# jnhansen/nd

Measured on AMD Instinct MI355X. Metric: Mpixels/s OmnibusTest dual-pol 24t x 4096 x 4096, higher is better.
Workload: dtype f32; 1 GPU; OmnibusTest C2 24t x 4096 x 4096 f32 per GPU (BASELINE configs[1]), resident in HBM; looks=9, rows_per_rank=4096

## Files before the change

nd_amd/build.py:

```python
import os
import subprocess
import sys

HERE = os.path.dirname(os.path.abspath(__file__))
CSRC = os.path.join(HERE, 'csrc')
OBJ = os.path.join(CSRC, '_build')
LIB = os.path.join(HERE, 'libnd_amd.so')
HIPCC = os.environ.get('HIPCC', '/opt/rocm/bin/hipcc')
ARCH = 'gfx950'

FLAGS = ['--offload-arch=' + ARCH, '-O3', '-std=c++17', '-fPIC', '-ffp-contract=off',
         '-fno-fast-math', '-Wall', '-Wno-unused-function']


PER_FILE = {'nlmeans.hip': ['-fno-slp-vectorize'],
            'omnibus.hip': ['-fno-slp-vectorize'],
            'omnibus_c3.hip': ['-fno-slp-vectorize'],
            'omnibus_ml.hip': ['-fno-slp-vectorize'],
            'omnibus_diag.hip': ['-fno-slp-vectorize']}


NO_SCRATCH = {'omnibus_ml.hip': 'omnibus_c2_ml_kernel', 'rgb.hip': 'rgb_', 'classify.hip': 'class',
              'kmeans_fit.hip': '_kernel', 'omnibus_diag.hip': 'omnibus_diag_',
              'change_segments.hip': 'change_segments_kernel', 'rasterize.hip': 'rasterize_', 'resample.hip': 'resample_',
              'speckle.hip': 'speckle_'}
SCRATCH_BUDGET = {(False, False): 0, (False, True): 96, (True, False): 256, (True, True): 384}


def _template_bools(mangled, symbol):
    import re
    m = re.search(re.escape(symbol) + r'I((?:L[ib]\d+E)+)E', mangled)
    if not m:
        return None
    flags = re.findall(r'Lb(\d)E', m.group(1))
    return (flags[0] == '1', flags[1] == '1') if len(flags) == 2 else None


def check_no_scratch(remarks_path, symbol, obj_path=None):
    import re
    if not os.path.exists(remarks_path) or (obj_path and os.path.exists(obj_path)
                                            and os.path.getmtime(remarks_path) + 1.0 < os.path.getmtime(obj_path)):
        return []
    found, cur = [], None
    for ln in open(remarks_path, errors='replace'):
        m = re.search(r'Function Name: (\S+)', ln)
        if m:
            cur = m.group(1)
            continue
        m = re.search(r'ScratchSize \[bytes/lane\]: (\d+)', ln)
        if m and cur is not None and symbol in cur:
            found.append((cur, int(m.group(1))))
    strict = os.environ.get('ND_AMD_STRICT_SCRATCH', '') == '1'
    if not found:
        msg = ('%s: no resource report for %s (is -Rpass-analysis=kernel-resource-usage on?)'
               % (remarks_path, symbol))
        if strict:
            raise RuntimeError(msg)
        sys.stderr.write('nd_amd.build: warning: ' + msg + '\n')
        return found
    bad = []
    for f, n in found:
        key = _template_bools(f, symbol)
        budget = SCRATCH_BUDGET.get(key, 0) if key is not None else 0
        if n > budget:
            bad.append((f, n, budget))
    if bad:
        msg = 'scratch use (bytes per lane) over budget: %s' % bad
        if strict:
            raise RuntimeError(msg)
        sys.stderr.write('nd_amd.build: warning: ' + msg + ' (speed only; ND_AMD_STRICT_SCRATCH=1 makes this an error)\n')
    return found


def sources():
    return sorted(os.path.join(CSRC, f) for f in os.listdir(CSRC) if f.endswith('.hip'))
# ... 71 lines not shown
```

nd_amd/csrc/omnibus.hip:

```cpp
#include <type_traits>

#include "dispatch.hpp"
#include "omnibus_c2_device.hpp"

namespace nd_amd {

template <typename T, int PPT, bool STATS>
__global__ void __launch_bounds__(kGlobalThreads)
omnibus_c2_global_kernel(const OmniGlobalArgs<T> g, const OmniTab tab)
{
    const int tid = threadIdx.x;
    const int lane = tid & 63;
    const int64_t b = blockIdx.x;
    const int64_t row = b / g.blocks_per_row;
    const int64_t bx = b - row * g.blocks_per_row;
    const int64_t bpx0 = bx * (int64_t)(kGlobalThreads * PPT);
    const int64_t x0 = bpx0 + (int64_t)tid * PPT;
    const int k = g.k;

    if (g.write_tab && b == 0) {
        for (int j = tid; j <= k; j += kGlobalThreads) g.tab_dev[j] = tab.e[j];
    }

    {
// ... 129 lines not shown
    const int64_t bpx0 = bx * (int64_t)kRetainThreads;
    const int64_t x0 = bpx0 + tid;
    const int k = g.k;
    const bool in = x0 < g.nx;

    T v[KMAX][4];
    retain_load_series<T, KMAX, EXACT>(g, row, bpx0, tid, in, k, v);

    if (g.write_tab && b == 0) {
        for (int j = tid; j <= k; j += kRetainThreads) g.tab_dev[j] = tab.e[j];
    }

    Accum<T> A;
    A.reset();
#pragma unroll
    for (int t = 0; t < KMAX; ++t)
        if (EXACT || t < k) A.step(v[t][0], v[t][1], v[t][2], v[t][3]);

    bool flag;
    if (STATS) {
        flag = global_flag_stats<T>(z_stat<T>(A, k, g.nlooks, g.e), 4 * (k - 1), g.e, g.alpha, in, g.z_out, g.p_out,
                                    row * g.nx + x0);
    } else {
        flag = in && (z_approx<T>(A, k, g.nlooks, g.e) >= g.e.zlo_a);
    }

    const unsigned long long m = __ballot(flag);
    const bool dense_wave = __popcll(m) >= g.dense_min;
    if (m != 0ull) {
        const unsigned shard = (unsigned)(b % kShards);
        if (dense_wave) {
            if (lane == 0) {
                const unsigned slot = atomicAdd(g.flag_count + shard * kCounterStride + 1, 1u);
                g.dense_idx[(size_t)shard * g.segd + slot] = (uint32_t)(row * g.nx + bpx0 + (tid & ~63));
            }
        } else {
            const unsigned slot = wave_claim(flag, g.flag_count + shard * kCounterStride, lane);
            if (flag) {
                g.flag_idx[(size_t)shard * g.seg + slot] = (uint32_t)(row * g.nx + x0);
                if (slot < g.dump_cap)
                    dump_series<T, KMAX, EXACT>(g.dump + ((int64_t)shard * g.dump_cap + slot) * (int64_t)(4 * k), v, k);
            }
        }
    }

    {
        const int64_t left = g.nx - bpx0;
        const int npx = left > kRetainThreads ? kRetainThreads : (int)left;
        zero_fill_span<kRetainThreads>(g.change + (row * g.nx + bpx0) * (int64_t)k, npx * k, tid);
    }
}

template <typename T, int KMAX, bool EXACT>
__global__ void __launch_bounds__(kRetainThreads, 4)
omnibus_c2_retain_wsearch_kernel(const OmniGlobalArgs<T> g, const OmniTab tab, const DenseScreen fscr)
{
    static_assert(KMAX % 4 == 0 && KMAX <= 24, "rows of whole words; 4 KMAX series registers within four waves per SIMD");
    constexpr int kWaves = kRetainThreads / 64;
    __shared__ __align__(16) T series_img[kWaves][kWaveSearchMax * KMAX * 4];
    __shared__ __align__(4) uint8_t rows_img[kWaves][kWaveSearchMax * KMAX];
    static_assert(sizeof(series_img[0]) >= 16 * KMAX * sizeof(uint32_t), "store_change_rows_wave's image");
    const int tid = threadIdx.x;
    const int lane = tid & 63;
    const int64_t b = blockIdx.x;
    const int64_t row = b / g.blocks_per_row;
    const int64_t bx = b - row * g.blocks_per_row;
    const int64_t bpx0 = bx * (int64_t)kRetainThreads;
    const int64_t x0 = bpx0 + tid;
    const int k = EXACT ? KMAX : g.k;
    const bool in = x0 < g.nx;

    T v[KMAX][4];
    retain_load_series<T, KMAX, EXACT>(g, row, bpx0, tid, in, k, v);

    if (g.write_tab && b == 0) {
        for (int j = tid; j <= k; j += kRetainThreads) g.tab_dev[j] = tab.e[j];
    }

    Accum<T> A;
    A.reset();
#pragma unroll
    for (int t = 0; t < KMAX; ++t)
        if (EXACT || t < k) A.step(v[t][0], v[t][1], v[t][2], v[t][3]);
    const bool flag = in && (z_approx<T>(A, k, g.nlooks, g.e) >= g.e.zlo_a);

    const unsigned long long m = __ballot(flag);
    const int nc = __popcll(m);
    const int64_t wpx0 = bpx0 + (tid & ~63);
    const int64_t wleft = g.nx - wpx0;
    const int wnp = wleft > 64 ? 64 : (wleft > 0 ? (int)wleft : 0);
    uint8_t *wob = g.change + (row * g.nx + wpx0) * (int64_t)k;

    if (nc == 0 || nc > kWaveSearchMax) {
        if (nc != 0 && lane == 0) {
            const unsigned shard = (unsigned)(b % kShards);
            const unsigned slot = atomicAdd(g.flag_count + shard * kCounterStride + 1, 1u);
            g.dense_idx[(size_t)shard * g.segd + slot] = (uint32_t)(row * g.nx + wpx0);
        }
        if (wnp > 0) zero_fill_span(wob, wnp * k, lane);
        return;
    }

    T *img = series_img[tid >> 6];
    uint8_t *rows = rows_img[tid >> 6];
    uint32_t *rows_w = reinterpret_cast<uint32_t *>(rows);
    const int rank = __popcll(m & ((1ull << lane) - 1ull));
    if (flag) dump_series<T, KMAX, EXACT>(img + rank * (KMAX * 4), v, k);
    for (int w = lane; w < kWaveSearchMax * KMAX / 4; w += 64) rows_w[w] = 0u;
    asm volatile("s_waitcnt lgkmcnt(0)" ::: "memory");
    wave_search_starts<T, KMAX>(img, rows, nc, k, g.nlooks, g.alpha, fscr.e, tab.e, lane);
    asm volatile("s_waitcnt lgkmcnt(0)" ::: "memory");
    unsigned mask = 0u;
    if (flag) {
#pragma unroll
        for (int q = 0; q < KMAX / 4; ++q)
            mask |= (((rows_w[rank * (KMAX / 4) + q] * 0x01020408u) >> 24) & 0xFu) << (4 * q);
    }
    if (change_rows_wave_ok(wob, k, wnp)) {
        store_change_rows_wave(wob, reinterpret_cast<uint32_t *>(img), k, mask, lane);
    } else if (in) {
        store_change_row_lane<KMAX>(wob + (int64_t)lane * k, k, mask);
    }
}

template <typename T, int KQ, int NS, bool STATS = false>
__global__ void __launch_bounds__(64 * NS)
omnibus_c2_split_kernel(const OmniGlobalArgs<T> g, const OmniTab tab, const float retain_rel)
{
    __shared__ T part_s[NS][4][64];
    __shared__ T fwd_s[STATS ? 4 : 1][64];
    __shared__ double fwd_p[64];
    __shared__ double part_p[NS][64];
    __shared__ int part_e[NS][3][64];
    __shared__ unsigned long long flag_mask;
    __shared__ unsigned list_base;
    const int tid = threadIdx.x, lane = tid & 63;
    const int w = __builtin_amdgcn_readfirstlane(tid >> 6);
    const int64_t b = blockIdx.x;
    const int64_t row = b / g.blocks_per_row;
    const int64_t bx = b - row * g.blocks_per_row;
    const int64_t gpx0 = bx * 64;
    const int64_t x0 = gpx0 + lane;
    const int k = g.k;
    const bool in = x0 < g.nx;
    const int t_lo = w * KQ;

    if (g.write_tab && b == 0)
        for (int j = tid; j <= k; j += 64 * NS) g.tab_dev[j] = tab.e[j];

    T v[KQ][4];
    {
        const int64_t ub = row * g.sy + gpx0;
        const unsigned lx = in ? (unsigned)lane : (unsigned)(g.nx - 1 - gpx0);
        const unsigned voff = lx * (unsigned)sizeof(T);
#pragma unroll
        for (int tt = 0; tt < KQ; ++tt) {
            const int t = t_lo + tt < k ? t_lo + tt : k - 1;
// ... 577 lines not shown
    const PV *i12i = reinterpret_cast<const PV *>(img + pm.img_off[2] + own * k);
    Accum<T> A;
    A.reset();
    const int nv = k / VE;
    for (int u = 0; u < nv; ++u) {
        const PV a = i11[u], d = i22[u];
        PV br, bi;
        if (JOINT) {
            const PV q0 = i12[2 * u], q1 = i12[2 * u + 1];
#pragma unroll
            for (int j = 0; j < VE; ++j) {
                br.v[j] = (j < VE / 2 ? q0 : q1).v[2 * (j % (VE / 2))];
                bi.v[j] = (j < VE / 2 ? q0 : q1).v[2 * (j % (VE / 2)) + 1];
            }
        } else {
            br = i12[u];
            bi = i12i[u];
        }
#pragma unroll
        for (int j = 0; j < VE; ++j) A.step(a.v[j], br.v[j], bi.v[j], d.v[j]);
    }

    bool flag;
    if (STATS) {
        flag = global_flag_stats<T>(z_stat<T>(A, k, g.nlooks, g.e), 4 * (k - 1), g.e, g.alpha, in, g.z_out, g.p_out, x0);
    } else {
        flag = in && (z_approx<T>(A, k, g.nlooks, g.e) >= g.e.zlo_a);
    }

    const unsigned shard = (unsigned)(b % kShards);
    if (__any(flag)) {
        const unsigned slot = wave_claim(flag, g.flag_count + shard * kCounterStride, lane);
        if (flag) g.flag_idx[(size_t)shard * g.seg + slot] = (uint32_t)x0;
    }
    zero_fill_span(g.change + px0 * (int64_t)k, np * k, lane);
}

template <typename T>
struct OmniDenseArgs {
    const T *c11, *c12r, *c12i, *c22;
    int64_t nx, npix;
    int64_t sy, sx, st;
    int k, flat;
    double nlooks, alpha;
    uint8_t *change;
    uint32_t *flag_count;
    const uint32_t *dense_idx;
    uint32_t segd;
    const OmniTabEntry *tab;
    uint32_t *flag_idx;
    uint32_t seg;
    T *dump;
    uint32_t dump_cap;
};



__device__ __forceinline__ void store_change_row(uint8_t *res, const int k, const unsigned long long mask)
{
    if ((k & 3) == 0 && ((uintptr_t)res & 3) == 0) {
        uint32_t *w = reinterpret_cast<uint32_t *>(res);
        for (int q = 0; q < (k >> 2); ++q) {
            const unsigned nib = (unsigned)(mask >> (4 * q)) & 0xFu;
            w[q] = (nib * 0x00204081u) & 0x01010101u;
        }
    } else {
        for (int t = 0; t < k; ++t) res[t] = (uint8_t)((mask >> t) & 1ull);
    }
}

template <typename T, int KMAX>
__global__ void __launch_bounds__(64, 2) omnibus_c2_dense_kernel(const OmniDenseArgs<T> s,
                                                              const StreamScreen<32> ss)
{
    __shared__ StreamEntry tab_lds[33];
    const int lane = threadIdx.x;
    const unsigned shard = blockIdx.x % kShards;
    const unsigned lblock = blockIdx.x / kShards, nlblock = gridDim.x / kShards;
    const uint32_t n = s.flag_count[shard * kCounterStride + 1];
    if (lblock >= n) return;
    const uint32_t *list = s.dense_idx + (size_t)shard * s.segd;
    if (lane <= 32) tab_lds[lane] = ss.e[lane];
    __syncthreads();

    for (uint32_t w = lblock; w < n; w += nlblock) {
        int k = s.k;
        asm volatile("" : "+s"(k));
        const int64_t pix0 = (int64_t)(uint32_t)__builtin_amdgcn_readfirstlane((int)list[w]);
        const int64_t pix = pix0 + lane;
        const int64_t row0 = pix0 / s.nx;
        const int64_t col0 = pix0 - row0 * s.nx;
        int64_t ub;
        unsigned delta;
        bool active;
        if (s.flat) {
            active = pix < s.npix;
            ub = pix0;
            delta = (unsigned)((active ? pix : s.npix - 1) - pix0);
        } else {
            active = col0 + lane < s.nx;
            ub = row0 * s.sy + col0 * s.sx;
            delta = (unsigned)(((active ? col0 + lane : s.nx - 1) - col0) * s.sx);
        }
        T v[KMAX][4];
#pragma unroll
        for (int t = 0; t < KMAX; ++t) {
            const int64_t ot = ub + (int64_t)(t < k ? t : k - 1) * s.st;
            v[t][0] = (s.c11 + ot)[delta];
            v[t][1] = (s.c12r + ot)[delta];
            v[t][2] = (s.c12i + ot)[delta];
            v[t][3] = (s.c22 + ot)[delta];
        }
        __builtin_amdgcn_sched_barrier(0);
        unsigned mask;
        bool handoff, cand;
        dense_chain<T, KMAX, 32>(v, k, active, ss, tab_lds, mask, handoff, cand);
        if (active && !handoff && mask != 0u) store_change_row(s.change + pix * (int64_t)k, k, mask);
        if (__any(handoff)) {
            const unsigned slot = wave_claim(handoff, s.flag_count + shard * kCounterStride, lane);
            if (handoff) {
                s.flag_idx[(size_t)shard * s.seg + slot] = (uint32_t)pix;
                if (slot < s.dump_cap)
                    dump_series<T, KMAX, false>(s.dump + ((int64_t)shard * s.dump_cap + slot) * (int64_t)(4 * k), v, k);
            }
        }
    }
}


template <typename T, int KMAX, bool EXACT, bool STATS = false>
__global__ void __launch_bounds__(kRetainThreads, chain_waves(KMAX, sizeof(T)))
omnibus_c2_chain_kernel(const OmniGlobalArgs<T> g, const OmniTab tab, const StreamScreen<chain_nj(KMAX)> ss)
{
    constexpr int NJ = chain_nj(KMAX);
    typedef typename std::conditional<(KMAX > 32), unsigned long long, unsigned>::type MT;
    if (omni_gate_skip(g)) return;
    __shared__ StreamEntry tab_lds[NJ + 1];
    __shared__ __align__(16) uint32_t out_img[(kRetainThreads / 64) * 16 * KMAX];
    const int tid = threadIdx.x;
    const int lane = tid & 63;
    const int64_t b = blockIdx.x;
    const int64_t row = b / g.blocks_per_row;
    const int64_t bx = b - row * g.blocks_per_row;
    const int64_t bpx0 = bx * (int64_t)kRetainThreads;
    const int64_t x0 = bpx0 + tid;
    const int k = EXACT ? KMAX : g.k;
    const bool in = x0 < g.nx;

    T v[KMAX][4];
    if (EXACT) {
        const int64_t ub = row * g.sy + bpx0;
        const unsigned lx = in ? (unsigned)tid : (unsigned)(g.nx - 1 - bpx0);
        const unsigned voff = lx * (unsigned)sizeof(T);
        const auto r11 = __builtin_amdgcn_make_buffer_rsrc(const_cast<T *>(g.c11 + ub), 0, 0x7fffffff, 0x00020000);
        const auto r12r = __builtin_amdgcn_make_buffer_rsrc(const_cast<T *>(g.c12r + ub), 0, 0x7fffffff, 0x00020000);
        const auto r12i = __builtin_amdgcn_make_buffer_rsrc(const_cast<T *>(g.c12i + ub), 0, 0x7fffffff, 0x00020000);
        const auto r22 = __builtin_amdgcn_make_buffer_rsrc(const_cast<T *>(g.c22 + ub), 0, 0x7fffffff, 0x00020000);
        const unsigned sstep = (unsigned)g.st * (unsigned)sizeof(T);
#pragma unroll
        for (int t = 0; t < KMAX; ++t) {
            const unsigned soff = (unsigned)t * sstep;
            v[t][0] = buffer_load<T>(r11, voff, soff);
            v[t][1] = buffer_load<T>(r12r, voff, soff);
            v[t][2] = buffer_load<T>(r12i, voff, soff);
            v[t][3] = buffer_load<T>(r22, voff, soff);
        }
    } else {
        const int64_t xc = in ? x0 : g.nx - 1;
        const int64_t off0 = row * g.sy + xc * g.sx;
#pragma unroll
        for (int t = 0; t < KMAX; ++t) {
            const int64_t off = off0 + (int64_t)(t < k ? t : k - 1) * g.st;
            v[t][0] = __builtin_nontemporal_load(g.c11 + off);
            v[t][1] = __builtin_nontemporal_load(g.c12r + off);
            v[t][2] = __builtin_nontemporal_load(g.c12i + off);
            v[t][3] = __builtin_nontemporal_load(g.c22 + off);
        }
// ... 1263 lines not shown
        const bool active = idx < n;
        const int64_t pix = active ? (int64_t)list[idx] : 0;
        T v[KMAX][4];
        if (idx < s.dump_cap) {
            const T *d = s.dump + ((int64_t)shard * s.dump_cap + idx) * (int64_t)(4 * k);
#pragma unroll
            for (int t = 0; t < KMAX; ++t) {
                const Pack<T, 4> q = *reinterpret_cast<const Pack<T, 4> *>(d + 4 * (t < k ? t : k - 1));
                v[t][0] = q.v[0];
                v[t][1] = q.v[1];
                v[t][2] = q.v[2];
                v[t][3] = q.v[3];
            }
        } else {
            const int64_t row = pix / s.nx;
            const int64_t col = pix - row * s.nx;
            const int64_t off = row * s.sy + col * s.sx;
            const T *p11 = s.c11 + off * s.m11, *p12r = s.c12r + off * s.m12;
            const T *p12i = s.c12i + off * s.m12, *p22 = s.c22 + off * s.m22;
            const int64_t d11 = s.st * s.m11, d12 = s.st * s.m12, d22 = s.st * s.m22;
#pragma unroll
            for (int t = 0; t < KMAX; ++t) {
                v[t][0] = *p11;
                v[t][1] = *p12r;
                v[t][2] = *p12i;
                v[t][3] = *p22;
                if (t < k - 1) {
                    p11 += d11;
                    p12r += d12;
                    p12i += d12;
                    p22 += d22;
                }
            }
        }
        unsigned cmask;
        bool handoff, cand;
        dense_chain<T, KMAX, 32>(v, k, active, ss, tab_lds, cmask, handoff, cand);
        {
            const unsigned long long hm = __ballot(handoff);
            if (lane == 0) {
                s.hand_bits[(size_t)shard * s.hand_words + (base >> 6)] = hm;
                if (hm != 0ull) atomicAdd(s.hand_count, (unsigned)__popcll(hm));
            }
        }
        if (active && !handoff) {
            uint8_t *res = s.change + pix * (int64_t)k;
            for (int u = 1; u < k; ++u)
                if ((cmask >> u) & 1u) res[u] = 1;
        }
    }
}

struct OmniWorkspace {
    size_t off_count, off_tab, off_idx, off_dense, off_hand, off_dump, min_total, recommended;
    uint32_t seg, segd, hand_words;
};

constexpr int kRetainMaxF32 = 48, kRetainMaxF64 = 24;
template <typename T>
constexpr bool retain_has(int kmax) { return kmax <= (sizeof(T) == 4 ? kRetainMaxF32 : kRetainMaxF64); }
template <typename T>
constexpr bool chain_has(int kmax) { return kmax <= (sizeof(T) == 4 ? 32 : 24); }
template <typename T>
constexpr bool dense_has(int kmax) { return kmax <= (sizeof(T) == 4 ? 32 : 16); }

constexpr size_t kCounterBytes = (size_t)kShards * kCounterStride * sizeof(uint32_t);

static uint32_t omni_seg(int64_t npix, int64_t ny)
{
    static_assert(kShards == 128, "bound below assumes 128 shards");
    const int64_t nb256 = ceil_div(npix, 256) + ny;
    return (uint32_t)(2 * nb256 + (2 * ny + 256) * 4 + 256);
}

static OmniWorkspace omni_layout(int64_t npix, int64_t ny, int64_t k, size_t elem, uint32_t seg_ml = 0)
{
    OmniWorkspace w;
    const uint32_t seg = seg_ml ? seg_ml : omni_seg(npix, ny);
    w.seg = seg;
    w.off_count = 0;
    w.off_tab = align256(kCounterBytes);
    w.off_idx = w.off_tab + align256((size_t)(k + 1) * sizeof(OmniTabEntry));
    w.off_dense = w.off_idx + align256((size_t)seg * kShards * sizeof(uint32_t));
    w.segd = seg / 64 + 8;
    w.off_hand = w.off_dense + align256((size_t)w.segd * kShards * sizeof(uint32_t));
    w.hand_words = seg / 64 + 1;
    w.off_dump = w.off_hand + align256((size_t)w.hand_words * kShards * sizeof(unsigned long long));
    w.min_total = w.off_dump;
    const size_t per = (size_t)k * 4 * elem;
    size_t cap = ((size_t)npix / 8 / kShards + 63) & ~(size_t)63;
    w.recommended = w.off_dump + align256(cap * kShards * per);
    if (seg_ml) {
        w.min_total = w.off_dump + align256((size_t)seg * kShards * per);
        w.recommended = w.min_total;
    }
    return w;
}

template <typename T>
static bool series_fits_buffer(const OmniGlobalArgs<T> &g)
{
    return g.sx == 1 && (int64_t)g.k * g.st * (int64_t)sizeof(T) < 0x7fffffffLL && g.st >= 0;
}

template <typename T, int PPT>
static void launch_global(const OmniGlobalArgs<T> &g, const OmniTab &tab, int64_t nblocks,
                          bool stats, hipStream_t stream)
{
    pick(stats, [&](auto S) {
        hipLaunchKernelGGL((omnibus_c2_global_kernel<T, PPT, decltype(S)::value>), dim3((unsigned)nblocks),
                           dim3(kGlobalThreads), 0, stream, g, tab);
    });
}

template <typename T>
static void launch_retain(const OmniGlobalArgs<T> &g, const OmniTab &tab, int64_t nblocks,
                          bool stats, hipStream_t stream)
{
    const dim3 grid((unsigned)nblocks), block(kRetainThreads);
    pick_le<8, 16, 24, 32, 48>(g.k, [&](auto K) {
        constexpr int KMAX = decltype(K)::value;
        if constexpr (retain_has<T>(KMAX))
            pick(g.k == KMAX && series_fits_buffer(g), [&](auto E) {
                pick(stats, [&](auto S) {
                    hipLaunchKernelGGL((omnibus_c2_retain_kernel<T, KMAX, decltype(E)::value, decltype(S)::value>),
                                       grid, block, 0, stream, g, tab);
                });
            });
    });
}

static bool wave_search_enabled()
{
    static const bool v = env_int("ND_AMD_WAVE_SEARCH", 1) != 0;
    return v;
}
static double fused_alpha_regs()
{
    static const double v = env_double("ND_AMD_FUSED_ALPHA", 0.93);
    return v;
}
constexpr int kWaveSearchMaxDates = 24;
constexpr double kWaveSearchAlpha = 0.99;
static bool omni_c2_wave_search(int dtype, int64_t k, int64_t stride_x, double alpha, uint32_t n_looks, bool stats)
{
    (void)stride_x;
    if (!wave_search_enabled() || dtype != ND_AMD_F32 || stats || n_looks == 0) return false;
    if (k < 2 || k > kWaveSearchMaxDates || !(alpha >= fused_alpha_regs()) || !(alpha >= kWaveSearchAlpha)) return false;
    const std::vector<OmniTabEntry> htab = get_table((int)k, n_looks, alpha, dtype, OmniFamily{2, 1});
    if (!((htab[(size_t)k].zlo > -INFINITY) || (htab[(size_t)k].zhi < INFINITY))) return false;
    const DenseScreen scr = make_dense_screen<float>(htab, (int)k, n_looks);
    for (int j = 2; j <= (int)k; ++j)
        if (!(scr.e[j].a > -INFINITY) && !(scr.e[j].b < INFINITY)) return false;
    return true;
}

template <typename T>
static void launch_retain_wsearch(const OmniGlobalArgs<T> &g, const OmniTab &tab, const DenseScreen &scr,
                                  int64_t nblocks, hipStream_t stream)
{
    if constexpr (std::is_same<T, float>::value) {
        const dim3 grid((unsigned)nblocks), block(kRetainThreads);
        pick_le<8, 16, kWaveSearchMaxDates>(g.k, [&](auto K) {
            constexpr int KMAX = decltype(K)::value;
            pick(g.k == KMAX && series_fits_buffer(g), [&](auto E) {
                hipLaunchKernelGGL((omnibus_c2_retain_wsearch_kernel<T, KMAX, decltype(E)::value>), grid, block, 0,
                                   stream, g, tab, scr);
            });
        });
    }
}

template <typename T>
static void launch_chain(const OmniGlobalArgs<T> &g, const OmniTab &tab, const std::vector<OmniTabEntry> &htab,
                         const DenseScreen &scr, uint32_t n_looks, int64_t nblocks, hipStream_t stream,
                         bool stats = false)
{
    const dim3 grid((unsigned)nblocks), block(kRetainThreads);
    const StreamScreen<32> ss = make_stream_screen<T, 32>(htab, scr, g.k, n_looks);
    pick_le<8, 16, 24, 32>(g.k, [&](auto K) {
        constexpr int KMAX = decltype(K)::value;
        if constexpr (chain_has<T>(KMAX))
            pick(g.k == KMAX && series_fits_buffer(g), [&](auto E) {
                pick(stats, [&](auto S) {
                    hipLaunchKernelGGL((omnibus_c2_chain_kernel<T, KMAX, decltype(E)::value, decltype(S)::value>),
                                       grid, block, 0, stream, g, tab, ss);
                });
            });
    });
}

static bool search_fs_enabled()
{
    static const bool v = env_int("ND_AMD_SEARCH_FS", 1) != 0;
    return v;
}

static int fused_form_env()
{
    static const int v = env_int("ND_AMD_FUSED_FORM", -1);
    return v;
}

template <typename T>
static int omnibus_c2_impl(const void *c11, const void *c12re, const void *c12im, const void *c22,
                           int64_t ny, int64_t nx, int64_t k, int64_t sy, int64_t sx, int64_t st,
                           uint32_t n_looks, double alpha, uint8_t *change, void *z_out,
                           void *p_out, void *workspace, size_t workspace_bytes,
                           hipStream_t stream, const int64_t *pm_ids = nullptr,
                           const OmniMlPlan *mlp = nullptr)
{
    const int64_t npix = ny * nx;
    const OmniWorkspace w = omni_layout(npix, ny, k, sizeof(T), mlp ? mlp->seg : 0);
    if (const int rc = check_workspace("nd_amd_omnibus_c2", workspace, workspace_bytes, w.min_total, true)) return rc;
    unsigned char *ws = static_cast<unsigned char *>(workspace);
    uint32_t *flag_count = reinterpret_cast<uint32_t *>(ws + w.off_count);
    OmniTabEntry *tab_dev = reinterpret_cast<OmniTabEntry *>(ws + w.off_tab);
    uint32_t *flag_idx = reinterpret_cast<uint32_t *>(ws + w.off_idx);

    const std::vector<OmniTabEntry> htab = get_table((int)k, n_looks, alpha, dtype_of<T>(), OmniFamily{2, 1});
    OmniTab tab;
    bool tab_in_args;
    ND_HIP_CHECK(stage_table(htab, k, &tab, tab_dev, stream, &tab_in_args));

    ND_HIP_CHECK(hipMemsetAsync(flag_count, 0, kCounterBytes, stream));

    OmniGlobalArgs<T> g;
    g.c11 = static_cast<const T *>(c11);
    g.c12r = static_cast<const T *>(c12re);
    g.c12i = static_cast<const T *>(c12im);
    g.c22 = static_cast<const T *>(c22);
    g.sy = sy;
    g.sx = sx;
    g.st = st;
    g.k = (int)k;
    g.write_tab = tab_in_args ? 1 : 0;
    g.nlooks = (double)n_looks;
    g.alpha = alpha;
    g.e = htab[(size_t)k];
    g.change = change;
    g.z_out = static_cast<T *>(z_out);
    g.p_out = static_cast<T *>(p_out);
    g.flag_count = flag_count;
    g.flag_idx = flag_idx;
    g.tab_dev = tab_dev;
    g.dense_idx = reinterpret_cast<uint32_t *>(ws + w.off_dense);
    g.segd = w.segd;
    const bool dense_ok = k <= (sizeof(T) == 4 ? 32 : 16) && pm_ids == nullptr && mlp == nullptr;
    g.dense_min = dense_ok ? kDenseMin : 65;
    const bool stats = (z_out != nullptr) || (p_out != nullptr);
    const bool retain = k <= (sizeof(T) == 4 ? kRetainMaxF32 : kRetainMaxF64);
    const bool global_screen_ok = (htab[(size_t)k].zlo > -INFINITY) || (htab[(size_t)k].zhi < INFINITY);
    const bool exact_flags = !global_screen_ok && mlp == nullptr && k >= 2;
    const bool stats_a = stats || exact_flags;
    static const double fused_alpha = env_double("ND_AMD_FUSED_ALPHA", 0.75);
    const double fused_alpha_regs = nd_amd::fused_alpha_regs();
    const bool fused = retain && dense_ok && alpha < fused_alpha_regs && !exact_flags;
    const bool fused_stats = fused && stats;
    const bool stream_long = !dense_ok && pm_ids == nullptr && mlp == nullptr && k <= kStreamChainMax &&
                             alpha < fused_alpha && !exact_flags;
    const bool ml_chain = mlp != nullptr && k >= 2 && alpha < fused_alpha_regs;
    static const bool stats_split_env0 = env_int("ND_AMD_STATS_SPLIT", 0) != 0;
    const bool stats_long_chain = stream_long && stats && !stats_split_env0 && k >= 3;
    const bool stats_split = stream_long && stats && !stats_long_chain;
    static const bool split_env = env_int("ND_AMD_C2_SPLIT", 1) != 0;
    const bool split_stats_ok = !(sizeof(T) == 8 && k > 48);
    const bool split_ok = split_env && search_fs_enabled() && !retain && !stream_long && (!stats || split_stats_ok) && !exact_flags &&
                          k <= (sizeof(T) == 4 ? 192 : 96) && pm_ids == nullptr && mlp == nullptr && sx == 1;
    static const bool gate_env = env_int("ND_AMD_GATE", 1) != 0;
    g.gate = flag_count + 2;
    g.gate_n = 0;
    g.gate_mode = 0;
    {
        const size_t per = (size_t)k * 4 * sizeof(T);
        size_t cap = (retain || stream_long || split_ok) ? (workspace_bytes - w.off_dump) / per / kShards : 0;
        g.seg = w.seg;
        if (cap > g.seg) cap = g.seg;
        if (split_ok) cap &= ~(size_t)63;
        g.dump = reinterpret_cast<T *>(ws + w.off_dump);
        g.dump_cap = (uint32_t)cap;
    }

    constexpr int VPPT = 16 / sizeof(T);
    const size_t es = sizeof(T);
    const bool aligned = (sx == 1) && (((uintptr_t)c11 | (uintptr_t)c12re | (uintptr_t)c12im |
                                        (uintptr_t)c22) & 15) == 0 &&
                         ((sy * (int64_t)es) % 16 == 0) && ((st * (int64_t)es) % 16 == 0);
    const bool flat = ((sx == 1) && (sy == nx)) || pm_ids != nullptr;
    g.nx = flat ? npix : nx;
    g.nrows = flat ? 1 : ny;
    unsigned long long *const hand_ws = reinterpret_cast<unsigned long long *>(ws + w.off_hand);
    const int ppt = retain ? 1 : (aligned ? VPPT : 1);
    g.blocks_per_row = ceil_div(g.nx, retain ? (int64_t)kRetainThreads : (int64_t)kGlobalThreads * ppt);
    const int64_t nblocks = g.blocks_per_row * g.nrows;
    if (nblocks > 0x7fffffffLL) {
        set_error("nd_amd_omnibus_c2: raster too large for one launch (%lld blocks)",
                  (long long)nblocks);
        return ND_AMD_EUNSUPPORTED;
    }
    auto take_sample = [&]() -> bool {
        const int64_t sblocks_total = ceil_div(npix, (int64_t)kRetainThreads);
        if (!gate_env || !retain || sblocks_total < 4096) return false;
        OmniSampleArgs<T> sa;
        sa.c11 = g.c11;
        sa.c12r = g.c12r;
        sa.c12i = g.c12i;
        sa.c22 = g.c22;
        sa.nx = g.nx;
        sa.blocks_per_row = ceil_div(g.nx, (int64_t)kRetainThreads);
        const int64_t total = sa.blocks_per_row * g.nrows;
        const int64_t nsb = pm_ids ? 128 : 512;
        sa.block_stride = total / nsb;
        sa.sy = sy;
        sa.sx = sx;
        sa.st = st;
        sa.m11 = pm_ids ? (int)pm_ids[0] : 1;
        sa.m12 = pm_ids ? (int)pm_ids[1] : 1;
        sa.m22 = pm_ids ? (int)pm_ids[3] : 1;
        sa.k = (int)k;
        sa.nlooks = g.nlooks;
        sa.e = g.e;
        sa.gate_out = flag_count + 2;
        g.gate_n = (uint32_t)(nsb * kRetainThreads);
        KernelTimer timer(ND_AMD_KERNEL_OMNIBUS_SAMPLE, stream);
        hipLaunchKernelGGL((omnibus_c2_sample_kernel<T>), dim3((unsigned)nsb), dim3(kRetainThreads), 0,
                           stream, sa);
        return true;
    };
    auto launch_dense = [&](hipStream_t sq, uint32_t *count, uint32_t *idx, uint32_t *dense_idx, T *dump,
                            uint32_t seg, uint32_t segd, uint32_t dump_cap, int64_t npix_listed) {
        OmniDenseArgs<T> d;
        d.c11 = g.c11;
        d.c12r = g.c12r;
        d.c12i = g.c12i;
        d.c22 = g.c22;
        d.nx = nx;
        d.npix = npix;
        d.sy = sy;
        d.sx = sx;
        d.st = st;
        d.k = (int)k;
        d.flat = flat ? 1 : 0;
        d.nlooks = g.nlooks;
        d.alpha = alpha;
        d.change = change;
        d.flag_count = count;
        d.dense_idx = dense_idx;
        d.segd = segd;
        d.tab = tab_dev;
        d.flag_idx = idx;
        d.seg = seg;
        d.dump = dump;
        d.dump_cap = dump_cap;
        int64_t per_shard_d = ceil_div(ceil_div(npix_listed, (int64_t)kShards), 64);
        if (per_shard_d > 32) per_shard_d = 32;
        if (per_shard_d < 1) per_shard_d = 1;
        const dim3 gridd((unsigned)(per_shard_d * kShards)), blockd(64);
        const DenseScreen scr = make_dense_screen<T>(htab, (int)k, n_looks);
        const StreamScreen<32> ssd = make_stream_screen<T, 32>(htab, scr, (int)k, n_looks);
        KernelTimer timer(ND_AMD_KERNEL_OMNIBUS_DENSE, sq);
        pick_le<8, 16, 24, 32>((int)k, [&](auto K) {
            constexpr int KMAX = decltype(K)::value;
            if constexpr (dense_has<T>(KMAX))
                hipLaunchKernelGGL((omnibus_c2_dense_kernel<T, KMAX>), gridd, blockd, 0, sq, d, ssd);
        });
    };
    const bool low_threshold = fused || stream_long || ml_chain || (pm_ids != nullptr && alpha < fused_alpha && !exact_flags);
    auto launch_search = [&](hipStream_t sq, const uint32_t *count, const uint32_t *idx, const T *dump,
                             uint32_t seg, uint32_t dump_cap, int64_t npix_listed,
                             unsigned long long *hand, uint32_t hand_words) -> int {
        OmniSearchArgs<T> s;
        s.c11 = g.c11;
        s.c12r = g.c12r;
        s.c12i = g.c12i;
        s.c22 = g.c22;
        s.nx = nx;
        s.sy = sy;
        s.sx = sx;
        s.st = st;
        s.m11 = pm_ids ? (int)pm_ids[0] : 1;
        s.m12 = pm_ids ? (int)pm_ids[1] : 1;
        s.m22 = pm_ids ? (int)pm_ids[3] : 1;
        s.k = (int)k;
        s.nlooks = g.nlooks;
        s.alpha = alpha;
        s.change = change;
        s.flag_count = count;
        s.flag_idx = idx;
        s.seg = seg;
        s.tab = tab_dev;
        s.dump = dump;
        s.dump_cap = dump_cap;
        s.hand_bits = nullptr;
        s.hand_words = hand_words;
        s.hand_count = const_cast<uint32_t *>(count) + 3;
        s.starts_max = 0;
        s.first = 0;
        const size_t scr_bytes = (size_t)(k + 1) * 4 * sizeof(double);
        const size_t lds_bytes = (size_t)k * 4 * 64 * sizeof(T) + scr_bytes;
        const bool use_lds = lds_bytes <= 150 * 1024;
        const bool fs = search_fs_enabled() && k <= kScreenLong;
        DenseScreenLong fscr;
        memset(&fscr, 0, sizeof(fscr));
        for (int j = 0; j <= kScreenLong; ++j) {
            fscr.e[j].a = -INFINITY;
            fscr.e[j].b = INFINITY;
// ... 390 lines not shown
                        pick(stats_long_chain, [&](auto S) {
                            hipLaunchKernelGGL((omnibus_c2_stream_chain_kernel<T, PF, decltype(B)::value ? 1 : 0, MW, decltype(S)::value>), grid, block, 0, stream, g, tab,
                                               make_stream_screen<T, NJ_>(htab, scr, (int)k, n_looks));
                        });
                    });
                });
            } else
                pick_le<32, 64, 128>((int)k, [&](auto NJ) {
                    constexpr int NJ_ = decltype(NJ)::value, MW = NJ_ / 64;
                    pick(buf, [&](auto B) {
                        hipLaunchKernelGGL((omnibus_c2_stream_kernel<T, PF, decltype(B)::value ? 1 : 0, MW>), grid, block, 0, stream, g, tab, nopm,
                                           make_stream_screen<T, NJ_>(htab, scr, (int)k, n_looks));
                    });
                });
            g.blocks_per_row = bpr_keep;
        }
        g.dense_min = 65;
        if (gated) {
            g.gate_mode = 2;
            KernelTimer timer(ND_AMD_KERNEL_OMNIBUS_GLOBAL, stream);
            launch_retain<T>(g, tab, nblocks, stats && !stats_split, stream);
        }
        g.gate_mode = 0;
    } else if (split_ok) {
        KernelTimer timer(ND_AMD_KERNEL_OMNIBUS_GLOBAL, stream);
        g.blocks_per_row = ceil_div(g.nx, (int64_t)64);
        const int64_t nbs = g.blocks_per_row * g.nrows;
        if (nbs > 0x7fffffffLL) {
            set_error("nd_amd_omnibus_c2: raster too large for one launch (%lld blocks)", (long long)nbs);
            return ND_AMD_EUNSUPPORTED;
        }
        const float rel = 3.f * (5.f * (float)k + 8.f) * (sizeof(T) == 4 ? 5.9604645e-08f : 1.1102230e-16f);
        const dim3 grid((unsigned)nbs);
        auto launch_split = [&](auto KQ, auto NS) {
            constexpr int NS_ = decltype(NS)::value;
            pick(stats, [&](auto S) {
                hipLaunchKernelGGL((omnibus_c2_split_kernel<T, decltype(KQ)::value, NS_, decltype(S)::value>), grid, dim3(64 * NS_), 0, stream,
                                   g, tab, rel);
            });
        };
        if constexpr (std::is_same<T, float>::value) {
            const int ns = k <= 96 ? 4 : 8;
            pick_eq<4, 8>(ns, [&](auto NS) {
                pick_le<16, 20, 24>((int)ceil_div(k, ns), [&](auto KQ) { launch_split(KQ, NS); });
            });
        } else {
            const int ns = k <= 48 ? 4 : 8;
            pick_eq<4, 8>(ns, [&](auto NS) {
                pick_le<8, 12>((int)ceil_div(k, ns), [&](auto KQ) { launch_split(KQ, NS); });
            });
        }
    } else {
        KernelTimer timer(ND_AMD_KERNEL_OMNIBUS_GLOBAL, stream);
        if (omni_c2_wave_search(dtype_of<T>(), k, sx, alpha, n_looks, stats) && g.dense_min == kDenseMin)
            launch_retain_wsearch<T>(g, tab, make_dense_screen<T>(htab, (int)k, n_looks), nblocks, stream);
        else if (retain)
            launch_retain<T>(g, tab, nblocks, stats || exact_flags, stream);
        else if (aligned)
            launch_global<T, VPPT>(g, tab, nblocks, stats || exact_flags, stream);
        else
            launch_global<T, 1>(g, tab, nblocks, stats || exact_flags, stream);
    }
    ND_HIP_CHECK(hipGetLastError());

    if (retain && g.dense_min <= 64 && (!fused || gated) && pm_ids == nullptr)
        launch_dense(stream, flag_count, flag_idx, g.dense_idx, g.dump, g.seg, g.segd, g.dump_cap, npix);
    ND_HIP_CHECK(hipGetLastError());

    {
        const int rc = launch_search(stream, flag_count, flag_idx, g.dump, g.seg, g.dump_cap, npix,
                                     hand_ws, g.seg / 64 + 1);
        if (rc != ND_AMD_OK) return rc;
    }
    ND_HIP_CHECK(hipGetLastError());
    return ND_AMD_OK;
}

}

using namespace nd_amd;

extern "C" size_t nd_amd_omnibus_c2_workspace_bytes(int dtype, int64_t ny, int64_t nx, int64_t k,
                                                    size_t *min_bytes)
{
    if (ny < 0 || nx < 0 || k < 0) return 0;
    const OmniWorkspace w = omni_layout(ny * nx, ny, k, dtype == ND_AMD_F64 ? 8 : 4);
    if (min_bytes) *min_bytes = w.min_total;
    return w.recommended;
}

extern "C" int nd_amd_omnibus_c2_uses_wave_search(int dtype, int64_t k, int64_t stride_x, double alpha,
                                                  uint32_t n_looks, int stats)
{
    return omni_c2_wave_search(dtype, k, stride_x, alpha, n_looks, stats != 0) ? 1 : 0;
}

extern "C" int nd_amd_omnibus_c2(const void *c11, const void *c12re, const void *c12im,
                                 const void *c22, int dtype, int64_t ny, int64_t nx, int64_t k,
                                 int64_t stride_y, int64_t stride_x, int64_t stride_t,
                                 uint32_t n_looks, double alpha, uint8_t *change, void *z_out,
                                 void *p_out, void *workspace, size_t workspace_bytes,
                                 void *hip_stream)
{
    if (dtype != ND_AMD_F32 && dtype != ND_AMD_F64) {
        set_error("nd_amd_omnibus_c2: dtype must be ND_AMD_F32 or ND_AMD_F64, got %d", dtype);
        return ND_AMD_EINVAL;
    }
    if (ny < 0 || nx < 0 || k < 0) {
        set_error("nd_amd_omnibus_c2: negative shape (%lld, %lld, %lld)", (long long)ny,
                  (long long)nx, (long long)k);
        return ND_AMD_EINVAL;
    }
    if (ny == 0 || nx == 0 || k == 0) return ND_AMD_OK;
    if (!c11 || !c12re || !c12im || !c22 || !change) {
        set_error("nd_amd_omnibus_c2: null data pointer");
        return ND_AMD_EINVAL;
    }
    if (n_looks == 0) {
        set_error("nd_amd_omnibus_c2: n_looks must be >= 1");
        return ND_AMD_EINVAL;
// ... 103 lines not shown
```

nd_amd/csrc/omnibus_c2_device.hpp:

```cpp
#pragma once
#include <type_traits>

#include "omnibus_common.hpp"
#include "omnibus_search.hpp"

namespace nd_amd {

template <typename T>
__device__ __forceinline__ T z_stat(const Accum<T> &A, int j, double nlooks, const OmniTabEntry &e)
{
    return z_stat(A, j, nlooks, e.m2rho, e.pklogk);
}
template <typename T>
__device__ __forceinline__ double z_approx(const Accum<T> &A, int j, double nlooks, const OmniTabEntry &e)
{
    return z_approx(A, j, nlooks, e.m2rho, e.pklogk);
}

constexpr int kNtAux = 2;

template <typename T>
__device__ __forceinline__ T buffer_load(__amdgpu_buffer_rsrc_t rsrc, unsigned voff, unsigned soff);
template <>
__device__ __forceinline__ float buffer_load<float>(__amdgpu_buffer_rsrc_t rsrc, unsigned voff,
                                                    unsigned soff)
{
    return __builtin_bit_cast(float, __builtin_amdgcn_raw_buffer_load_b32(rsrc, voff, soff, kNtAux));
}
template <>
__device__ __forceinline__ double buffer_load<double>(__amdgpu_buffer_rsrc_t rsrc, unsigned voff,
                                                      unsigned soff)
{
    return __builtin_bit_cast(double, __builtin_amdgcn_raw_buffer_load_b64(rsrc, voff, soff, kNtAux));
}

template <typename T, int N>
struct alignas(sizeof(T) * N) Pack {
    T v[N];
};

template <typename T, int KMAX, bool EXACT>
__device__ __forceinline__ void dump_series(T *d, const T (&v)[KMAX][4], const int k)
{
#pragma unroll
    for (int t = 0; t < KMAX; ++t) {
        if (EXACT || t < k) {
            Pack<T, 4> q;
            q.v[0] = v[t][0];
            q.v[1] = v[t][1];
            q.v[2] = v[t][2];
            q.v[3] = v[t][3];
            *reinterpret_cast<Pack<T, 4> *>(d + 4 * t) = q;
        }
    }
}

template <typename T>
struct OmniGlobalArgs {
    const T *c11, *c12r, *c12i, *c22;
    int64_t nx, nrows;
    int64_t sy, sx, st;
    int64_t blocks_per_row;
    int k;
    int write_tab;
    double nlooks, alpha;
    OmniTabEntry e;
    uint8_t *change;
    T *z_out, *p_out;
    uint32_t *flag_count;
    uint32_t *flag_idx;
    uint32_t seg;
    OmniTabEntry *tab_dev;
    T *dump;
    uint32_t dump_cap;
    uint32_t *dense_idx;
    uint32_t segd;
    int dense_min;
    const uint32_t *gate;
    uint32_t gate_n;
    int gate_mode;
};

template <typename T>
__device__ __forceinline__ bool omni_gate_skip(const OmniGlobalArgs<T> &g)
{
    if (g.gate_mode == 0) return false;
    const uint32_t hits = __builtin_nontemporal_load(g.gate);
    const bool dense = hits * 8u >= g.gate_n;
    return (g.gate_mode == 1) != dense;
}

constexpr int kGlobalThreads = 256;
constexpr int kRetainThreads = 256;
constexpr int kShards = 128;
constexpr int kCounterStride = 32;
constexpr int kTimeChunk = 4;

template <typename T, int KMAX, bool EXACT>
__device__ __forceinline__ void retain_load_series(const OmniGlobalArgs<T> &g, const int64_t row, const int64_t bpx0,
                                                   const int tid, const bool in, const int k, T (&v)[KMAX][4])
{
    if (EXACT) {
        const int64_t ub = row * g.sy + bpx0;
        const unsigned lx = in ? (unsigned)tid : (unsigned)(g.nx - 1 - bpx0);
        const unsigned voff = lx * (unsigned)sizeof(T);
        const auto r11 = __builtin_amdgcn_make_buffer_rsrc(const_cast<T *>(g.c11 + ub), 0, 0x7fffffff, 0x00020000);
        const auto r12r = __builtin_amdgcn_make_buffer_rsrc(const_cast<T *>(g.c12r + ub), 0, 0x7fffffff, 0x00020000);
        const auto r12i = __builtin_amdgcn_make_buffer_rsrc(const_cast<T *>(g.c12i + ub), 0, 0x7fffffff, 0x00020000);
        const auto r22 = __builtin_amdgcn_make_buffer_rsrc(const_cast<T *>(g.c22 + ub), 0, 0x7fffffff, 0x00020000);
        const unsigned sstep = (unsigned)g.st * (unsigned)sizeof(T);
#pragma unroll
        for (int t = 0; t < KMAX; ++t) {
            const unsigned soff = (unsigned)t * sstep;
            v[t][0] = buffer_load<T>(r11, voff, soff);
            v[t][1] = buffer_load<T>(r12r, voff, soff);
            v[t][2] = buffer_load<T>(r12i, voff, soff);
            v[t][3] = buffer_load<T>(r22, voff, soff);
        }
    } else {
        const int64_t xc = in ? bpx0 + tid : g.nx - 1;
        const int64_t off0 = row * g.sy + xc * g.sx;
#pragma unroll
        for (int t = 0; t < KMAX; ++t) {
            if (t < k) {
                const int64_t off = off0 + (int64_t)t * g.st;
                v[t][0] = __builtin_nontemporal_load(g.c11 + off);
                v[t][1] = __builtin_nontemporal_load(g.c12r + off);
                v[t][2] = __builtin_nontemporal_load(g.c12i + off);
                v[t][3] = __builtin_nontemporal_load(g.c22 + off);
            }
        }
    }
}

template <int KMAX, typename MT>
__device__ __forceinline__ void store_change_row_lane(uint8_t *res, const int k, const MT mask)
{
    if ((k & 3) == 0 && ((uintptr_t)res & 3) == 0) {
        uint32_t *w = reinterpret_cast<uint32_t *>(res);
#pragma unroll
        for (int q = 0; q < KMAX / 4; ++q)
            if (q < (k >> 2)) w[q] = (mask_nibble(mask, q) * 0x00204081u) & 0x01010101u;
    } else {
        for (int t = 0; t < k; ++t) res[t] = (uint8_t)((mask >> t) & (MT)1);
    }
}
// ... 182 lines not shown
```

Baseline: 14310 Mpixels/s.

## Split wave-search kernel into single-wave workgroups with XCD-aware mapping and flag-map dense pass

The retain wave-search kernel now launches one 64-thread workgroup per wave instead of 256-thread blocks. Workgroup ids are remapped so the four waves of a 256-pixel block spread across XCDs. Instead of atomically appending dense-wave indices to sharded lists, each wave writes a byte flag. A new dense map kernel scans these flags and processes marked waves directly, which removes the flag-count memset, the atomics and the later search launch on this path. The cost is a larger grid of small workgroups, a flag-array scan over all waves, and extra LDS per workgroup.

Measured after the change: 14280 Mpixels/s. No clear change (-0.2%).

```diff
diff --git a/nd_amd/build.py b/nd_amd/build.py
--- a/nd_amd/build.py
+++ b/nd_amd/build.py
@@ -20,7 +20,8 @@
             'omnibus_diag.hip': ['-fno-slp-vectorize']}
 
 
-NO_SCRATCH = {'omnibus_ml.hip': 'omnibus_c2_ml_kernel', 'rgb.hip': 'rgb_', 'classify.hip': 'class',
+NO_SCRATCH = {'omnibus.hip': 'omnibus_c2_retain_wsearch_kernel',
+              'omnibus_ml.hip': 'omnibus_c2_ml_kernel', 'rgb.hip': 'rgb_', 'classify.hip': 'class',
               'kmeans_fit.hip': '_kernel', 'omnibus_diag.hip': 'omnibus_diag_',
               'change_segments.hip': 'change_segments_kernel', 'rasterize.hip': 'rasterize_', 'resample.hip': 'resample_',
               'speckle.hip': 'speckle_'}
diff --git a/nd_amd/csrc/omnibus.hip b/nd_amd/csrc/omnibus.hip
--- a/nd_amd/csrc/omnibus.hip
+++ b/nd_amd/csrc/omnibus.hip
@@ -205,17 +205,19 @@
 }
 
 template <typename T, int KMAX, bool EXACT>
-__global__ void __launch_bounds__(kRetainThreads, 4)
+__global__ void __launch_bounds__(64, 4)
 omnibus_c2_retain_wsearch_kernel(const OmniGlobalArgs<T> g, const OmniTab tab, const DenseScreen fscr)
 {
     static_assert(KMAX % 4 == 0 && KMAX <= 24, "rows of whole words; 4 KMAX series registers within four waves per SIMD");
-    constexpr int kWaves = kRetainThreads / 64;
-    __shared__ __align__(16) T series_img[kWaves][kWaveSearchMax * KMAX * 4];
-    __shared__ __align__(4) uint8_t rows_img[kWaves][kWaveSearchMax * KMAX];
-    static_assert(sizeof(series_img[0]) >= 16 * KMAX * sizeof(uint32_t), "store_change_rows_wave's image");
-    const int tid = threadIdx.x;
-    const int lane = tid & 63;
-    const int64_t b = blockIdx.x;
+    __shared__ __align__(16) T series_img[kWaveSearchMax * KMAX * 4];
+    __shared__ __align__(4) uint8_t rows_img[kWaveSearchMax * KMAX];
+    static_assert(sizeof(series_img) >= 16 * KMAX * sizeof(uint32_t), "store_change_rows_wave's image");
+    const int lane = threadIdx.x;
+    const int64_t id = blockIdx.x;
+    const int64_t vw = (id & ~(int64_t)31) + (id & 7) * kWsearchWaves + ((id & 31) >> 3);
+    const int64_t b = vw / kWsearchWaves;
+    if (b >= g.blocks_per_row * g.nrows) return;
+    const int tid = (int)(vw % kWsearchWaves) * 64 + lane;
     const int64_t row = b / g.blocks_per_row;
     const int64_t bx = b - row * g.blocks_per_row;
     const int64_t bpx0 = bx * (int64_t)kRetainThreads;
@@ -226,8 +228,8 @@
     T v[KMAX][4];
     retain_load_series<T, KMAX, EXACT>(g, row, bpx0, tid, in, k, v);
 
-    if (g.write_tab && b == 0) {
-        for (int j = tid; j <= k; j += kRetainThreads) g.tab_dev[j] = tab.e[j];
+    if (g.write_tab && vw == 0) {
+        for (int j = lane; j <= k; j += 64) g.tab_dev[j] = tab.e[j];
     }
 
     Accum<T> A;
@@ -244,18 +246,15 @@
     const int wnp = wleft > 64 ? 64 : (wleft > 0 ? (int)wleft : 0);
     uint8_t *wob = g.change + (row * g.nx + wpx0) * (int64_t)k;
 
+    if (lane == 0) g.wave_flags[vw] = (uint8_t)(nc > kWaveSearchMax ? 1 : 0);
+
     if (nc == 0 || nc > kWaveSearchMax) {
-        if (nc != 0 && lane == 0) {
-            const unsigned shard = (unsigned)(b % kShards);
-            const unsigned slot = atomicAdd(g.flag_count + shard * kCounterStride + 1, 1u);
-            g.dense_idx[(size_t)shard * g.segd + slot] = (uint32_t)(row * g.nx + wpx0);
-        }
         if (wnp > 0) zero_fill_span(wob, wnp * k, lane);
         return;
     }
 
-    T *img = series_img[tid >> 6];
-    uint8_t *rows = rows_img[tid >> 6];
+    T *img = series_img;
+    uint8_t *rows = rows_img;
     uint32_t *rows_w = reinterpret_cast<uint32_t *>(rows);
     const int rank = __popcll(m & ((1ull << lane) - 1ull));
     if (flag) dump_series<T, KMAX, EXACT>(img + rank * (KMAX * 4), v, k);
@@ -939,6 +938,8 @@
     uint32_t seg;
     T *dump;
     uint32_t dump_cap;
+    const uint8_t *wave_flags;
+    int64_t nwaves, waves_per_row;
 };
 
 
@@ -954,6 +955,37 @@
     } else {
         for (int t = 0; t < k; ++t) res[t] = (uint8_t)((mask >> t) & 1ull);
     }
+}
+
+template <typename T, int KMAX>
+__device__ __forceinline__ bool dense_load_wave(const OmniDenseArgs<T> &s, const int k, const int64_t pix0,
+                                                const int lane, T (&v)[KMAX][4])
+{
+    const int64_t pix = pix0 + lane;
+    const int64_t row0 = pix0 / s.nx;
+    const int64_t col0 = pix0 - row0 * s.nx;
+    int64_t ub;
+    unsigned delta;
+    bool active;
+    if (s.flat) {
+        active = pix < s.npix;
+        ub = pix0;
+        delta = (unsigned)((active ? pix : s.npix - 1) - pix0);
+    } else {
+        active = col0 + lane < s.nx;
+        ub = row0 * s.sy + col0 * s.sx;
+        delta = (unsigned)(((active ? col0 + lane : s.nx - 1) - col0) * s.sx);
+    }
+#pragma unroll
+    for (int t = 0; t < KMAX; ++t) {
+        const int64_t ot = ub + (int64_t)(t < k ? t : k - 1) * s.st;
+        v[t][0] = (s.c11 + ot)[delta];
+        v[t][1] = (s.c12r + ot)[delta];
+        v[t][2] = (s.c12i + ot)[delta];
+        v[t][3] = (s.c22 + ot)[delta];
+    }
+    __builtin_amdgcn_sched_barrier(0);
+    return active;
 }
 
 template <typename T, int KMAX>
@@ -975,30 +1007,8 @@
         asm volatile("" : "+s"(k));
         const int64_t pix0 = (int64_t)(uint32_t)__builtin_amdgcn_readfirstlane((int)list[w]);
         const int64_t pix = pix0 + lane;
-        const int64_t row0 = pix0 / s.nx;
-        const int64_t col0 = pix0 - row0 * s.nx;
-        int64_t ub;
-        unsigned delta;
-        bool active;
-        if (s.flat) {
-            active = pix < s.npix;
-            ub = pix0;
-            delta = (unsigned)((active ? pix : s.npix - 1) - pix0);
-        } else {
-            active = col0 + lane < s.nx;
-            ub = row0 * s.sy + col0 * s.sx;
-            delta = (unsigned)(((active ? col0 + lane : s.nx - 1) - col0) * s.sx);
-        }
         T v[KMAX][4];
-#pragma unroll
-        for (int t = 0; t < KMAX; ++t) {
-            const int64_t ot = ub + (int64_t)(t < k ? t : k - 1) * s.st;
-            v[t][0] = (s.c11 + ot)[delta];
-            v[t][1] = (s.c12r + ot)[delta];
-            v[t][2] = (s.c12i + ot)[delta];
-            v[t][3] = (s.c22 + ot)[delta];
-        }
-        __builtin_amdgcn_sched_barrier(0);
+        const bool active = dense_load_wave<T, KMAX>(s, k, pix0, lane, v);
         unsigned mask;
         bool handoff, cand;
         dense_chain<T, KMAX, 32>(v, k, active, ss, tab_lds, mask, handoff, cand);
@@ -1010,6 +1020,66 @@
                 if (slot < s.dump_cap)
                     dump_series<T, KMAX, false>(s.dump + ((int64_t)shard * s.dump_cap + slot) * (int64_t)(4 * k), v, k);
             }
+        }
+    }
+}
+
+template <typename T, int KMAX>
+__global__ void __launch_bounds__(64, 2) omnibus_c2_dense_map_kernel(const OmniDenseArgs<T> s,
+                                                                  const StreamScreen<32> ss, const DenseScreen fscr)
+{
+    static_assert(KMAX % 4 == 0 && KMAX <= 32, "rows of whole words, masks of 32 bits");
+    __shared__ StreamEntry tab_lds[33];
+    __shared__ __align__(16) T series_img[kWaveSearchMax * KMAX * 4];
+    __shared__ __align__(4) uint8_t rows_img[kWaveSearchMax * KMAX];
+    uint32_t *rows_w = reinterpret_cast<uint32_t *>(rows_img);
+    const int lane = threadIdx.x;
+    bool staged = false;
+    for (int64_t w0 = (int64_t)blockIdx.x * 64; w0 < s.nwaves; w0 += (int64_t)gridDim.x * 64) {
+        const bool marked = (w0 + lane < s.nwaves) && s.wave_flags[w0 + lane] != 0;
+        unsigned long long todo = __ballot(marked);
+        if (todo == 0ull) continue;
+        if (!staged) {
+            if (lane <= 32) tab_lds[lane] = ss.e[lane];
+            __syncthreads();
+            staged = true;
+        }
+        while (todo != 0ull) {
+            const int64_t w = w0 + (__ffsll(todo) - 1);
+            todo &= todo - 1ull;
+            int k = s.k;
+            asm volatile("" : "+s"(k));
+            int64_t pix0 = w * 64;
+            if (!s.flat) {
+                const int64_t row0 = w / s.waves_per_row;
+                pix0 = row0 * s.nx + (w - row0 * s.waves_per_row) * 64;
+            }
+            const int64_t pix = pix0 + lane;
+            T v[KMAX][4];
+            const bool active = dense_load_wave<T, KMAX>(s, k, pix0, lane, v);
+            unsigned mask;
+            bool handoff, cand;
+            dense_chain<T, KMAX, 32>(v, k, active, ss, tab_lds, mask, handoff, cand);
+            unsigned long long hm = __ballot(handoff);
+            while (hm != 0ull) {
+                const int rank = __popcll(hm & ((1ull << lane) - 1ull));
+                const bool mine = ((hm >> lane) & 1ull) && rank < kWaveSearchMax;
+                const int nh = __popcll(hm);
+                if (mine) dump_series<T, KMAX, false>(series_img + rank * (KMAX * 4), v, k);
+                for (int q = lane; q < kWaveSearchMax * KMAX / 4; q += 64) rows_w[q] = 0u;
+                asm volatile("s_waitcnt lgkmcnt(0)" ::: "memory");
+                wave_search_starts<T, KMAX>(series_img, rows_img, nh < kWaveSearchMax ? nh : kWaveSearchMax, k, s.nlooks,
+                                            s.alpha, fscr.e, s.tab, lane);
+                asm volatile("s_waitcnt lgkmcnt(0)" ::: "memory");
+                if (mine) {
+                    mask = 0u;
+#pragma unroll
+                    for (int q = 0; q < KMAX / 4; ++q)
+                        mask |= (((rows_w[rank * (KMAX / 4) + q] * 0x01020408u) >> 24) & 0xFu) << (4 * q);
+                }
+                hm &= ~__ballot(mine);
+            }
+            if (active && mask != 0u) store_change_row(s.change + pix * (int64_t)k, k, mask);
         }
     }
 }
@@ -2379,7 +2449,7 @@
 }
 
 struct OmniWorkspace {
-    size_t off_count, off_tab, off_idx, off_dense, off_hand, off_dump, min_total, recommended;
+    size_t off_count, off_tab, off_idx, off_dense, off_hand, off_wflag, off_dump, min_total, recommended;
     uint32_t seg, segd, hand_words;
 };
 
@@ -2412,7 +2482,8 @@
     w.segd = seg / 64 + 8;
     w.off_hand = w.off_dense + align256((size_t)w.segd * kShards * sizeof(uint32_t));
     w.hand_words = seg / 64 + 1;
-    w.off_dump = w.off_hand + align256((size_t)w.hand_words * kShards * sizeof(unsigned long long));
+    w.off_wflag = w.off_hand + align256((size_t)w.hand_words * kShards * sizeof(unsigned long long));
+    w.off_dump = w.off_wflag + align256((size_t)(ceil_div(npix, (int64_t)kRetainThreads) + ny) * (kRetainThreads / 64));
     w.min_total = w.off_dump;
     const size_t per = (size_t)k * 4 * elem;
     size_t cap = ((size_t)npix / 8 / kShards + 63) & ~(size_t)63;
@@ -2487,7 +2558,7 @@
                                   int64_t nblocks, hipStream_t stream)
 {
     if constexpr (std::is_same<T, float>::value) {
-        const dim3 grid((unsigned)nblocks), block(kRetainThreads);
+        const dim3 grid((unsigned)(ceil_div(nblocks * kWsearchWaves, (int64_t)32) * 32)), block(64);
         pick_le<8, 16, kWaveSearchMaxDates>(g.k, [&](auto K) {
             constexpr int KMAX = decltype(K)::value;
             pick(g.k == KMAX && series_fits_buffer(g), [&](auto E) {
@@ -2549,8 +2620,6 @@
     OmniTab tab;
     bool tab_in_args;
     ND_HIP_CHECK(stage_table(htab, k, &tab, tab_dev, stream, &tab_in_args));
-
-    ND_HIP_CHECK(hipMemsetAsync(flag_count, 0, kCounterBytes, stream));
 
     OmniGlobalArgs<T> g;
     g.c11 = static_cast<const T *>(c11);
@@ -2594,6 +2663,12 @@
     const bool split_stats_ok = !(sizeof(T) == 8 && k > 48);
     const bool split_ok = split_env && search_fs_enabled() && !retain && !stream_long && (!stats || split_stats_ok) && !exact_flags &&
                           k <= (sizeof(T) == 4 ? 192 : 96) && pm_ids == nullptr && mlp == nullptr && sx == 1;
+    const bool wsearch = mlp == nullptr && pm_ids == nullptr && dense_ok && !fused && !stream_long && !split_ok &&
+                         omni_c2_wave_search(dtype_of<T>(), k, sx, alpha, n_looks, stats);
+    if (!wsearch) ND_HIP_CHECK(hipMemsetAsync(flag_count, 0, kCounterBytes, stream));
+    g.wave_flags = ws + w.off_wflag;
+    DenseScreen scr_w;
+    if (wsearch) scr_w = make_dense_screen<T>(htab, (int)k, n_looks);
     static const bool gate_env = env_int("ND_AMD_GATE", 1) != 0;
     g.gate = flag_count + 2;
     g.gate_n = 0;
@@ -2679,6 +2754,21 @@
         d.seg = seg;
         d.dump = dump;
         d.dump_cap = dump_cap;
+        d.wave_flags = g.wave_flags;
+        d.nwaves = nblocks * kWsearchWaves;
+        d.waves_per_row = g.blocks_per_row * kWsearchWaves;
+        if (wsearch) {
+            int64_t nb = ceil_div(d.nwaves, (int64_t)64);
+            if (nb > 4096) nb = 4096;
+            const StreamScreen<32> ssd = make_stream_screen<T, 32>(htab, scr_w, (int)k, n_looks);
+            KernelTimer timer(ND_AMD_KERNEL_OMNIBUS_DENSE, sq);
+            if constexpr (std::is_same<T, float>::value)
+                pick_le<8, 16, kWaveSearchMaxDates>((int)k, [&](auto K) {
+                    hipLaunchKernelGGL((omnibus_c2_dense_map_kernel<T, decltype(K)::value>), dim3((unsigned)nb), dim3(64), 0,
+                                       sq, d, ssd, scr_w);
+                });
+            return;
+        }
         int64_t per_shard_d = ceil_div(ceil_div(npix_listed, (int64_t)kShards), 64);
         if (per_shard_d > 32) per_shard_d = 32;
         if (per_shard_d < 1) per_shard_d = 1;
@@ -3175,8 +3265,8 @@
         }
     } else {
         KernelTimer timer(ND_AMD_KERNEL_OMNIBUS_GLOBAL, stream);
-        if (omni_c2_wave_search(dtype_of<T>(), k, sx, alpha, n_looks, stats) && g.dense_min == kDenseMin)
-            launch_retain_wsearch<T>(g, tab, make_dense_screen<T>(htab, (int)k, n_looks), nblocks, stream);
+        if (wsearch)
+            launch_retain_wsearch<T>(g, tab, scr_w, nblocks, stream);
         else if (retain)
             launch_retain<T>(g, tab, nblocks, stats || exact_flags, stream);
         else if (aligned)
@@ -3189,6 +3279,7 @@
     if (retain && g.dense_min <= 64 && (!fused || gated) && pm_ids == nullptr)
         launch_dense(stream, flag_count, flag_idx, g.dense_idx, g.dump, g.seg, g.segd, g.dump_cap, npix);
     ND_HIP_CHECK(hipGetLastError());
+    if (wsearch) return ND_AMD_OK;
 
     {
         const int rc = launch_search(stream, flag_count, flag_idx, g.dump, g.seg, g.dump_cap, npix,
diff --git a/nd_amd/csrc/omnibus_c2_device.hpp b/nd_amd/csrc/omnibus_c2_device.hpp
--- a/nd_amd/csrc/omnibus_c2_device.hpp
+++ b/nd_amd/csrc/omnibus_c2_device.hpp
@@ -76,6 +76,7 @@
     uint32_t *dense_idx;
     uint32_t segd;
     int dense_min;
+    uint8_t *wave_flags;
     const uint32_t *gate;
     uint32_t gate_n;
     int gate_mode;
@@ -92,6 +93,8 @@
 
 constexpr int kGlobalThreads = 256;
 constexpr int kRetainThreads = 256;
+constexpr int kWsearchWaves = kRetainThreads / 64;
+static_assert(kWsearchWaves == 4, "the kernel's XCD mapping: 8 XCDs x 4 waves to a group of 32 workgroups");
 constexpr int kShards = 128;
 constexpr int kCounterStride = 32;
 constexpr int kTimeChunk = 4;
```
